# CreateIntelligens/index-tts-lora

Measured on AMD Instinct MI355X. Metric: audio-seconds/sec (RTF^-1) at batch 32, whole pipeline (GPT decode + latent pass + BigVGAN), higher is better.
Workload: dtype bf16; 1 GPU; BASELINE config 3: batch=32 utterances/GPU, top-k sampling (k=30,p=0.8), 140 acoustic tokens (5.97 s) each, shared 3.2 s prompt, text U{20..60} tokens, random-init weights at real shapes; gpt_dtype=bf16, vocoder_dtype=fp16, parallelism=dp1 (utterance sharding, no collectives), schedule=serial: one batch at a time on one stream

## Files before the change

index-tts-lora_amd/csrc/attention.hip:

```cpp
#include "common.h"
#include <type_traits>

namespace itts {

constexpr int HD = 64;

constexpr int AD_MAXCTX = 16384;
constexpr int AD_CH = 8;

__device__ __forceinline__ void softmax_merge(float& m, float& l, float m2, float l2, float& sa, float& sb) {
  float M = fmaxf(m, m2);
  sa = (m == -INFINITY) ? 0.f : __expf(m - M);
  sb = (m2 == -INFINITY) ? 0.f : __expf(m2 - M);
  l = l * sa + l2 * sb;
  m = M;
}

template <typename T, int NWV, bool IND, bool PAGED>
__global__ __launch_bounds__(NWV * 64) void attn_decode_kernel(const T* __restrict__ q, const T* __restrict__ kc,
                                                           const T* __restrict__ vc, T* __restrict__ out,
                                                           const int32_t* __restrict__ pad, const int32_t* __restrict__ pos,
                                                           int H, int smax, int out_mtp, const int32_t* __restrict__ kv_rows,
                                                           const int32_t* __restrict__ kv_step, int rows_total,
                                                           const int32_t* __restrict__ skip_rows,
                                                           const int32_t* __restrict__ kv_share,
                                                           const int32_t* __restrict__ kv_tab, int bs_log2) {
  typedef Elem<T> EL;
  typedef typename EL::frag frag;
  constexpr int E = EL::E;
  constexpr int LPR = HD / E;

  constexpr int RPW = 64 / LPR;
  constexpr int CH = AD_CH * 4 / NWV;
  __shared__ float w_m[NWV], w_l[NWV];
  __shared__ float w_o[NWV][HD];
  const int h = blockIdx.x, b = blockIdx.y;
  const int tid = threadIdx.x, lane = tid & 63, wave = tid >> 6;
  const int part = lane % LPR, rg = lane / LPR;
  const frag qv = ld16<frag>(q + ((int64_t)b * H + h) * HD + part * E);
  int tabv = 0, tab0v = 0;
  if constexpr (PAGED) {
    tabv = kv_tab[b * ITTS_KV_TAB + lane];
    tab0v = kv_tab[lane];
  }
  const int bsm = (1 << bs_log2) - 1;
  const int32_t* skip_ptr = skip_rows != nullptr ? skip_rows + b : pos;
  const int skip_raw = *skip_ptr;
  const int j0 = pad[b];
  const bool skipped = skip_rows != nullptr && skip_raw != 0;
  const int32_t* share_ptr = kv_share != nullptr ? kv_share : pos;
  const int share_raw = *share_ptr;
  const int share_w = (kv_share != nullptr && !IND) ? share_raw : 0;
  const int shC = share_w & 255;
  int pos0 = pos[0];
  asm volatile("" : "+s"(pos0));
  const int ctx = skipped ? j0 : pos0 + 1;
  const T* kb = kc + (PAGED ? 0 : ((int64_t)b * H + h) * smax * HD) + part * E;
  const T* vb = vc + (PAGED ? 0 : ((int64_t)b * H + h) * smax * HD) + part * E;
  const int64_t sh_off = ((int64_t)h * smax + (share_w >> 8)) * HD + part * E;
  const int32_t* tab = nullptr;
  if constexpr (IND) tab = kv_rows + ((int64_t)(kv_step[0] & 1) * rows_total + b) * smax;

  float qf[E];
  float m = -INFINITY, l = 0.f, o[E];
#pragma unroll
  for (int e = 0; e < E; ++e) o[e] = 0.f;

  const int wave_u = __builtin_amdgcn_readfirstlane(wave);
  auto key_pass = [&](const int base, auto first_tag) {
    constexpr bool FIRST = decltype(first_tag)::value;
    frag kf[CH], vf[CH];
    int prow[CH];
    if constexpr (IND) {
#pragma unroll
      for (int i = 0; i < CH; ++i) {
        int j = min(base + (i * NWV + wave) * RPW + rg, ctx - 1);
        prow[i] = tab[j];
      }
    }
#pragma unroll
    for (int i = 0; i < CH; ++i) {
      const int jf = min(base + (i * NWV + wave_u) * RPW, (ctx - 1) & ~(RPW - 1));
      int j = min(jf + rg, ctx - 1);
      int64_t ro = (int64_t)j * HD;
      if constexpr (IND) ro += (int64_t)(prow[i] - b) * H * smax * HD;
      if constexpr (PAGED) {
        const int blk = __builtin_amdgcn_readlane(tabv, (jf >> bs_log2) & (ITTS_KV_TAB - 1));
        ro = ((((int64_t)blk * H + h) << bs_log2) + (j & bsm)) * HD;
      }
      const T* kp = kb + ro;
      const T* vp = vb + ro;
      if constexpr (!IND) {
        const bool sh = (unsigned)(j - j0) < (unsigned)shC;
        int64_t so = sh_off + (int64_t)(j - j0) * HD;
        if constexpr (PAGED) {
          const int ps = (share_w >> 8) + (j - j0);
          const int blk0 = __shfl(tab0v, (ps >> bs_log2) & (ITTS_KV_TAB - 1), 64);
          so = ((((int64_t)blk0 * H + h) << bs_log2) + (ps & bsm)) * HD + part * E;
        }
        kp = sh ? kc + so : kp;
        vp = sh ? vc + so : vp;
      }
      kf[i] = ld16<frag>(kp);
      vf[i] = ld16<frag>(vp);
    }
    __builtin_amdgcn_sched_barrier(0);
    if constexpr (FIRST) {
#pragma unroll
      for (int e = 0; e < E; ++e) qf[e] = EL::to_f(qv[e]) * 0.125f;
      __builtin_amdgcn_sched_barrier(0);
    }
    float sc[CH];
    float cmax = -INFINITY;
#pragma unroll
    for (int i = 0; i < CH; ++i) {
      float d = 0.f;
#pragma unroll
      for (int e = 0; e < E; ++e) d = fmaf(qf[e], EL::to_f(kf[i][e]), d);
#pragma unroll
      for (int off = 1; off < LPR; off <<= 1) d += __shfl_xor(d, off, 64);
      int j = base + (i * NWV + wave) * RPW + rg;
      sc[i] = (j >= j0 && j < ctx) ? d : -INFINITY;
      cmax = fmaxf(cmax, sc[i]);
    }
    {
      const float M = fmaxf(m, cmax);
      const float Ms = (M == -INFINITY) ? 0.f : M;
      const float corr = (m == -INFINITY) ? 0.f : __expf(m - Ms);
      l *= corr;
#pragma unroll
      for (int e = 0; e < E; ++e) o[e] *= corr;
#pragma unroll
      for (int i = 0; i < CH; ++i) {
        float pv = __expf(sc[i] - Ms);
        l += pv;
#pragma unroll
        for (int e = 0; e < E; ++e) o[e] = fmaf(pv, EL::to_f(vf[i][e]), o[e]);
      }
      m = M;
    }
  };
  constexpr int PASS = 4 * RPW * AD_CH;
  if (j0 < ctx) {
    const int b0 = j0 & ~(RPW - 1);
    key_pass(b0, std::true_type{});
    for (int base = b0 + PASS; base < ctx; base += PASS) key_pass(base, std::false_type{});
  }
#pragma unroll
  for (int off = LPR; off < 64; off <<= 1) {
    float m2 = __shfl_xor(m, off, 64), l2 = __shfl_xor(l, off, 64);
    float sa, sb;
    softmax_merge(m, l, m2, l2, sa, sb);
#pragma unroll
    for (int e = 0; e < E; ++e) {
      float o2 = __shfl_xor(o[e], off, 64);
      o[e] = o[e] * sa + o2 * sb;
    }
  }
  if (rg == 0) {
#pragma unroll
    for (int e = 0; e < E; ++e) w_o[wave][part * E + e] = o[e];
    if (part == 0) {
      w_m[wave] = m;
      w_l[wave] = l;
    }
  }
  __syncthreads();
  if (tid < HD && !skipped) {
    float M = w_m[0];
#pragma unroll
    for (int w = 1; w < NWV; ++w) M = fmaxf(M, w_m[w]);
    float L = 0.f, acc = 0.f;
#pragma unroll
    for (int w = 0; w < NWV; ++w) {
      float sw = (w_m[w] == -INFINITY) ? 0.f : __expf(w_m[w] - M);
      L += w_l[w] * sw;
      acc += w_o[w][tid] * sw;
    }
    const int64_t o = out_mtp > 0 ? pa_off<T>(b, h * HD + tid, out_mtp) : ((int64_t)b * H + h) * HD + tid;
    out[o] = EL::from_f(L > 0.f ? acc / L : 0.f);
  }
}

template <typename T>
__global__ __launch_bounds__(256) void attn_prefill_kernel(const T* __restrict__ qkv, T* __restrict__ out,
                                                            T* __restrict__ kc, T* __restrict__ vc,
                                                            const int32_t* __restrict__ pad, int S, int H, int smax,
                                                            const int32_t* __restrict__ row_off,
                                                            const int32_t* __restrict__ cache_shift,
                                                            const T* __restrict__ pkc, const T* __restrict__ pvc,
                                                            const int32_t* __restrict__ pre_len,
                                                            const int32_t* __restrict__ pre_row,
                                                            const int32_t* __restrict__ pre_pos0, int pre_qkv,
                                                            T* wkc, T* wvc, const int32_t* __restrict__ w_row,
                                                            const int32_t* __restrict__ w_pos0,
                                                            const int32_t* __restrict__ kv_tab, int bs_log2) {
  typedef Elem<T> EL;
  typedef typename EL::frag frag;
  constexpr int E = EL::E, KS = EL::KS, NKS = HD / KS;
  constexpr int ES = (int)sizeof(T);
  constexpr int RS = HD * ES + 16;
  constexpr int CPR = HD / E;
  __shared__ __attribute__((aligned(16))) unsigned char Ks[64 * RS];
  __shared__ __attribute__((aligned(16))) unsigned char Vt[64 * RS];
  __shared__ __attribute__((aligned(16))) unsigned char Ps[4][16 * RS];
  const int q0 = blockIdx.x * 64, h = blockIdx.y, b = blockIdx.z;
  const int tid = threadIdx.x, lane = tid & 63, wave = tid >> 6;
  const int g = lane >> 4, c = lane & 15;
  const int D = H * HD;
  const int rbeg = row_off ? row_off[b] : b * S;
  if (row_off) S = row_off[b + 1] - rbeg;
  if (q0 >= S) return;
  const int cshift = (row_off && cache_shift) ? cache_shift[b] : 0;
  const int j0 = (pad && !row_off) ? pad[b] : 0;
  const T* base = qkv + (int64_t)rbeg * 3 * D;
  const int pl = pkc != nullptr ? pre_len[b] : 0;
  const int64_t pstr = pre_qkv ? (int64_t)3 * D : HD;
  const int64_t pbase = pkc == nullptr ? 0
                        : pre_qkv      ? (int64_t)pre_pos0[b] * 3 * D + h * HD
                                       : (((int64_t)pre_row[b] * H + h) * smax + pre_pos0[b]) * HD;
  const int p_row = (pkc != nullptr && !pre_qkv) ? pre_row[b] : 0, p_pos0 = (pkc != nullptr && !pre_qkv) ? pre_pos0[b] : 0;
  const int Stot = pl + S;
  if (wkc != nullptr) {
    const int wr = w_row[b], wp0 = w_pos0[b];
    for (int ch = tid; ch < 64 * CPR; ch += 256) {
      const int kk = ch / CPR, dc = ch - kk * CPR;
      const int q = q0 + kk;
      if (q < S) {
        const T* src = base + (int64_t)q * 3 * D + D + h * HD + dc * E;
        const int64_t o = kv_elem_off(kv_tab, bs_log2, wr, wp0 + q, H, h, smax) + dc * E;
        st16(wkc + o, ld16<frag>(src));
        st16(wvc + o, ld16<frag>(src + D));
      }
    }
  }

  frag qf[NKS];
  {
    const int row = q0 + wave * 16 + c;
#pragma unroll
    for (int ks = 0; ks < NKS; ++ks)
      qf[ks] = (row < S) ? ld16<frag>(base + (int64_t)row * 3 * D + h * HD + ks * KS + g * E) : zero_frag<frag>();
  }
  f32x4 O[4];
#pragma unroll
  for (int n = 0; n < 4; ++n) O[n] = f32x4{0.f, 0.f, 0.f, 0.f};
  float m[4], l[4];
#pragma unroll
  for (int j = 0; j < 4; ++j) { m[j] = -INFINITY; l[j] = 0.f; }

  const int jend = min(Stot, pl + q0 + 64);
  for (int jt = (j0 / 64) * 64; jt < jend; jt += 64) {
    __syncthreads();
    for (int ch = tid; ch < 64 * CPR; ch += 256) {
      const int kk = ch / CPR, dc = ch - kk * CPR;
      const int key = jt + kk;
      frag kv = zero_frag<frag>(), vv = zero_frag<frag>();
      if (key < pl) {
        const int64_t po = (kv_tab != nullptr && !pre_qkv) ? kv_elem_off(kv_tab, bs_log2, p_row, p_pos0 + key, H, h, smax) + dc * E
                                                           : pbase + (int64_t)key * pstr + dc * E;
        kv = ld16<frag>(pkc + po);
        vv = ld16<frag>(pvc + po);
      } else if (key < Stot) {
        const T* src = base + (int64_t)(key - pl) * 3 * D + D + h * HD + dc * E;
        kv = ld16<frag>(src);
        vv = ld16<frag>(src + D);
        if (kc != nullptr && jt == q0) {
          const int64_t o = kv_elem_off(kv_tab, bs_log2, b, key + cshift, H, h, smax) + dc * E;
          st16(kc + o, kv);
          st16(vc + o, vv);
        }
      }
      st16(Ks + kk * RS + dc * E * ES, kv);
#pragma unroll
      for (int e = 0; e < E; ++e) *reinterpret_cast<T*>(Vt + (dc * E + e) * RS + kk * ES) = vv[e];
    }
    __syncthreads();
    if (jt + 64 <= j0) continue;
    f32x4 sacc[4];
#pragma unroll
    for (int n = 0; n < 4; ++n) {
      sacc[n] = f32x4{0.f, 0.f, 0.f, 0.f};
#pragma unroll
      for (int ks = 0; ks < NKS; ++ks) {
        frag bf = ld16<frag>(Ks + (16 * n + c) * RS + (ks * KS + g * E) * ES);
        sacc[n] = EL::mma(qf[ks], bf, sacc[n]);
      }
    }
    float rmax[4];
#pragma unroll
    for (int j = 0; j < 4; ++j) {
      const int q = pl + q0 + wave * 16 + 4 * g + j;
      float mx = -INFINITY;
#pragma unroll
      for (int n = 0; n < 4; ++n) {
        const int key = jt + 16 * n + c;
        const bool vis = (key <= q) && (key >= j0) && (key < Stot);
        const float v = vis ? sacc[n][j] * 0.125f : -INFINITY;
        sacc[n][j] = v;
        mx = fmaxf(mx, v);
      }
#pragma unroll
      for (int o = 1; o < 16; o <<= 1) mx = fmaxf(mx, __shfl_xor(mx, o, 64));
      rmax[j] = mx;
    }
#pragma unroll
    for (int j = 0; j < 4; ++j) {
      const float mn = fmaxf(m[j], rmax[j]);
      const float corr = (m[j] == -INFINITY) ? 0.f : __expf(m[j] - mn);
      float rs = 0.f;
#pragma unroll
      for (int n = 0; n < 4; ++n) {
        const float pv = (sacc[n][j] == -INFINITY) ? 0.f : __expf(sacc[n][j] - mn);
        sacc[n][j] = pv;
        rs += pv;
      }
#pragma unroll
      for (int o = 1; o < 16; o <<= 1) rs += __shfl_xor(rs, o, 64);
      l[j] = l[j] * corr + rs;
      m[j] = mn;
#pragma unroll
      for (int n = 0; n < 4; ++n) O[n][j] *= corr;
    }
    unsigned char* ps = Ps[wave];
#pragma unroll
    for (int n = 0; n < 4; ++n)
#pragma unroll
      for (int j = 0; j < 4; ++j) *reinterpret_cast<T*>(ps + (4 * g + j) * RS + (16 * n + c) * ES) = EL::from_f(sacc[n][j]);
#pragma unroll
    for (int ks = 0; ks < NKS; ++ks) {
      frag af = ld16<frag>(ps + c * RS + (ks * KS + g * E) * ES);
#pragma unroll
      for (int n = 0; n < 4; ++n) {
        frag bf = ld16<frag>(Vt + (16 * n + c) * RS + (ks * KS + g * E) * ES);
        O[n] = EL::mma(af, bf, O[n]);
      }
    }
  }
#pragma unroll
  for (int j = 0; j < 4; ++j) {
    const int q = q0 + wave * 16 + 4 * g + j;
    if (q >= S) continue;
    const float inv = l[j] > 0.f ? 1.0f / l[j] : 0.f;
    T* orow = out + ((int64_t)rbeg + q) * D + h * HD;
#pragma unroll
    for (int n = 0; n < 4; ++n) orow[16 * n + c] = EL::from_f(O[n][j] * inv);
  }
}

}

using namespace itts;

#if ITTS_DIAG
namespace itts { int g_attn_waves = 4; }
#else
namespace itts { constexpr int g_attn_waves = 4; }
#endif

extern "C" int itts_attn_decode(const void* q, const void* kcache, const void* vcache, void* out, const int32_t* pad,
                                const int32_t* pos, int B, int H, int smax, int dtype, int out_packed, const int32_t* kv_rows,
                                const int32_t* kv_step, const int32_t* skip_rows, const int32_t* kv_share, const int32_t* kv_tab,
                                int kv_bs, void* stream) {
  const int out_mtp = out_packed ? (B + 15) / 16 : 0;
  ITTS_REQUIRE(q && kcache && vcache && out && pad && pos, "itts_attn_decode: null pointer");
  const bool paged = kv_tab != nullptr;
  ITTS_REQUIRE(B > 0 && H > 0 && (paged || (smax > 0 && smax <= AD_MAXCTX)), "itts_attn_decode: bad shape B=%d H=%d smax=%d (max %d)", B, H,
               smax, AD_MAXCTX);
  ITTS_REQUIRE(!paged || ((kv_bs == 16 || kv_bs == 32 || kv_bs == 64) && kv_rows == nullptr),
               "itts_attn_decode: a paged cache needs kv_bs in {16, 32, 64} and no beam row table");
  const int bs_log2 = kv_bs == 64 ? 6 : kv_bs == 32 ? 5 : 4;
  ITTS_REQUIRE((kv_rows == nullptr) == (kv_step == nullptr), "itts_attn_decode: pass both or neither of kv_rows / kv_step");
  hipStream_t s = (hipStream_t)stream;
  dim3 grid(H, B), block(g_attn_waves * 64);
  const bool ind = kv_rows != nullptr;
#define ITTS_AD(TT_, NW_, IND_, PG_)                                                                                        \
  hipLaunchKernelGGL((attn_decode_kernel<TT_, NW_, IND_, PG_>), grid, block, 0, s, (const TT_*)q, (const TT_*)kcache,      \
                     (const TT_*)vcache, (TT_*)out, pad, pos, H, smax, out_mtp, kv_rows, kv_step, B, skip_rows, kv_share, \
                     kv_tab, bs_log2)
#define ITTS_AD_T(TT_)                                                            \
  do {                                                                            \
    if (paged) { if (g_attn_waves == 8) ITTS_AD(TT_, 8, false, true); else ITTS_AD(TT_, 4, false, true); } \
    else if (g_attn_waves == 8) { if (ind) ITTS_AD(TT_, 8, true, false); else ITTS_AD(TT_, 8, false, false); } \
    else { if (ind) ITTS_AD(TT_, 4, true, false); else ITTS_AD(TT_, 4, false, false); }          \
  } while (0)
  switch (dtype) {
    case ITTS_F32:
      ITTS_AD_T(float);
      break;
    case ITTS_BF16:
      ITTS_AD_T(bf16_t);
      break;
    case ITTS_F16:
      ITTS_AD_T(f16_t);
      break;
    default:
      ITTS_REQUIRE(false, "itts_attn_decode: unknown dtype %d", dtype);
  }
#undef ITTS_AD_T
#undef ITTS_AD
  return check_launch("itts_attn_decode");
}

static int attn_prefill_impl(const void* qkv, void* out, void* kcache, void* vcache, const int32_t* pad, int B, int S, int H,
                             int smax, int dtype, const int32_t* row_off, const int32_t* cache_shift, void* stream,
                             const void* pkc = nullptr, const void* pvc = nullptr, const int32_t* pre_len = nullptr,
                             const int32_t* pre_row = nullptr, const int32_t* pre_pos0 = nullptr, int pre_qkv = 0,
                             void* wkc = nullptr, void* wvc = nullptr, const int32_t* w_row = nullptr,
                             const int32_t* w_pos0 = nullptr, const int32_t* kv_tab = nullptr, int kv_bs = 0) {
  ITTS_REQUIRE(qkv && out, "itts_attn_prefill: null pointer");
  ITTS_REQUIRE(kv_tab == nullptr || kv_bs == 16 || kv_bs == 32 || kv_bs == 64, "itts_attn_prefill: kv_bs must be 16, 32 or 64");
  const int bs_log2 = kv_bs == 64 ? 6 : kv_bs == 32 ? 5 : 4;
  if (kv_tab != nullptr && kcache != nullptr) smax = S > smax ? S : smax;
  ITTS_REQUIRE((kcache == nullptr) == (vcache == nullptr), "itts_attn_prefill: pass both caches or neither");
  ITTS_REQUIRE(B > 0 && S > 0 && H > 0 && (!kcache || S <= smax), "itts_attn_prefill: bad shape B=%d S=%d H=%d smax=%d", B, S, H, smax);
  ITTS_REQUIRE(B <= 65535 && H <= 65535, "itts_attn_prefill: grid too large");
  dim3 grid((S + 63) / 64, H, B), block(256);
  hipStream_t s = (hipStream_t)stream;
  switch (dtype) {
    case ITTS_F32:
      hipLaunchKernelGGL(attn_prefill_kernel<float>, grid, block, 0, s, (const float*)qkv, (float*)out, (float*)kcache, (float*)vcache, pad, S, H, smax, row_off, cache_shift,
                         (const float*)pkc, (const float*)pvc, pre_len, pre_row, pre_pos0, pre_qkv, (float*)wkc, (float*)wvc, w_row, w_pos0, kv_tab, bs_log2);
      break;
    case ITTS_BF16:
      hipLaunchKernelGGL(attn_prefill_kernel<bf16_t>, grid, block, 0, s, (const bf16_t*)qkv, (bf16_t*)out, (bf16_t*)kcache, (bf16_t*)vcache, pad, S, H, smax, row_off, cache_shift,
                         (const bf16_t*)pkc, (const bf16_t*)pvc, pre_len, pre_row, pre_pos0, pre_qkv, (bf16_t*)wkc, (bf16_t*)wvc, w_row, w_pos0, kv_tab, bs_log2);
      break;
    case ITTS_F16:
      hipLaunchKernelGGL(attn_prefill_kernel<f16_t>, grid, block, 0, s, (const f16_t*)qkv, (f16_t*)out, (f16_t*)kcache, (f16_t*)vcache, pad, S, H, smax, row_off, cache_shift,
                         (const f16_t*)pkc, (const f16_t*)pvc, pre_len, pre_row, pre_pos0, pre_qkv, (f16_t*)wkc, (f16_t*)wvc, w_row, w_pos0, kv_tab, bs_log2);
      break;
    default:
      ITTS_REQUIRE(false, "itts_attn_prefill: unknown dtype %d", dtype);
  }
  return check_launch("itts_attn_prefill");
}

extern "C" int itts_attn_prefill(const void* qkv, void* out, void* kcache, void* vcache, const int32_t* pad, int B, int S,
                                 int H, int smax, int dtype, void* stream) {
  return attn_prefill_impl(qkv, out, kcache, vcache, pad, B, S, H, smax, dtype, nullptr, nullptr, stream);
}

extern "C" int itts_attn_prefill_prefix(const void* qkv, void* out, const void* kcache, const void* vcache, const int32_t* row_off,
                                        const int32_t* pre_len, const int32_t* pre_row, const int32_t* pre_pos0, int B, int Smax,
                                        int H, int smax, int dtype, const int32_t* kv_tab, int kv_bs, void* stream) {
  ITTS_REQUIRE(row_off && kcache && vcache && pre_len && pre_row && pre_pos0, "itts_attn_prefill_prefix: null pointer");
  return attn_prefill_impl(qkv, out, nullptr, nullptr, nullptr, B, Smax, H, smax, dtype, row_off, nullptr, stream, kcache, vcache,
                           pre_len, pre_row, pre_pos0, 0, nullptr, nullptr, nullptr, nullptr, kv_tab, kv_bs);
}

extern "C" int itts_attn_prefill_shared(const void* qkv, void* out, void* kcache, void* vcache, const int32_t* row_off,
                                        const int32_t* pre_len, const int32_t* pre_row0, const int32_t* w_row,
                                        const int32_t* w_pos0, int E, int Smax, int H, int smax, int dtype, const int32_t* kv_tab,
                                        int kv_bs, void* stream) {
  ITTS_REQUIRE(qkv && row_off && pre_len && pre_row0 && (kcache == nullptr) == (vcache == nullptr) &&
                   (kcache == nullptr || (w_row && w_pos0)), "itts_attn_prefill_shared: null pointer");
  const int D = H * 64;
  const int es = dtype == ITTS_F32 ? 4 : 2;
  const char* q = (const char*)qkv;
  return attn_prefill_impl(qkv, out, nullptr, nullptr, nullptr, E, Smax, H, smax, dtype, row_off, nullptr, stream,
                           q + (int64_t)D * es, q + (int64_t)2 * D * es, pre_len, pre_len , pre_row0, 1, kcache, vcache,
                           w_row, w_pos0, kv_tab, kv_bs);
}

extern "C" int itts_attn_prefill_packed(const void* qkv, void* out, void* kcache, void* vcache, const int32_t* row_off,
                                        const int32_t* cache_shift, int B, int Smax, int H, int smax, int dtype,
                                        const int32_t* kv_tab, int kv_bs, void* stream) {
  ITTS_REQUIRE(row_off, "itts_attn_prefill_packed: row_off is null");
  return attn_prefill_impl(qkv, out, kcache, vcache, nullptr, B, Smax, H, smax, dtype, row_off, cache_shift, stream, nullptr, nullptr,
                           nullptr, nullptr, nullptr, 0, nullptr, nullptr, nullptr, nullptr, kv_tab, kv_bs);
}

namespace itts {
__global__ __launch_bounds__(256) void kv_share_rows_kernel(char* __restrict__ kc, char* __restrict__ vc, int64_t layer_bytes, int H, int C,
                                                            int p0, const int32_t* __restrict__ pad, int smax,
                                                            const int32_t* __restrict__ kv_tab, int bs_log2, int es, int total) {
  const int idx = (int)blockIdx.x * 256 + threadIdx.x;
  if (idx >= total) return;
  const int cpr = 64 * es / 16;
  const int seg = idx % cpr, kv = (idx / cpr) & 1, rest = idx / (2 * cpr);
  const int c = rest % C, h = rest / C;
  const int b = (int)blockIdx.y + 1;
  char* base = (kv ? vc : kc) + (int64_t)blockIdx.z * layer_bytes;
  const int64_t so = kv_elem_off(kv_tab, bs_log2, 0, p0 + c, H, h, smax) * es + seg * 16;
  const int64_t d_o = kv_elem_off(kv_tab, bs_log2, b, pad[b] + c, H, h, smax) * es + seg * 16;
  st16(base + d_o, ld16<B16>(base + so));
}
}

extern "C" int itts_kv_share_rows(void* kcache, void* vcache, int layers, int64_t layer_stride, int B, int H, int C, int p0,
                                  const int32_t* pad, int smax, const int32_t* kv_tab, int kv_bs, int dtype, void* stream) {
  ITTS_REQUIRE(kcache && vcache && pad && layers > 0 && B >= 1 && H > 0 && C > 0 && p0 >= 0, "itts_kv_share_rows: bad arguments");
  ITTS_REQUIRE(kv_tab != nullptr ? (kv_bs == 16 || kv_bs == 32 || kv_bs == 64) : smax >= p0 + C,
               "itts_kv_share_rows: paged cache: kv_bs must be 16, 32 or 64; contiguous cache: smax covers the block");
  ITTS_REQUIRE(layers <= 65535 && B <= 65536, "itts_kv_share_rows: too many layers / rows");
  if (B == 1) return ITTS_OK;
  const int es = dtype == ITTS_F32 ? 4 : 2;
  const int total = H * C * 2 * (64 * es / 16);
  hipLaunchKernelGGL(itts::kv_share_rows_kernel, dim3((total + 255) / 256, B - 1, layers), dim3(256), 0, (hipStream_t)stream, (char*)kcache,
                     (char*)vcache, layer_stride * es, H, C, p0, pad, smax, kv_tab, kv_bs == 64 ? 6 : kv_bs == 32 ? 5 : 4, es, total);
  return itts::check_launch("itts_kv_share_rows");
}
```

index-tts-lora_amd/csrc/gemm_skinny.hip:

```cpp
#include "common.h"
#include "ln_math.h"
#include <type_traits>

#ifndef ITTS_FOLD_ORDER
#define ITTS_FOLD_ORDER 0
#endif
#ifndef ITTS_NT_WEIGHTS
#define ITTS_NT_WEIGHTS 0
#endif

namespace itts {

template <typename F>
__device__ __forceinline__ F ldw(const void* p) {
  if constexpr (ITTS_NT_WEIGHTS) return ld16_nt<F>(p);
  else return ld16<F>(p);
}

struct SkinnyParams {
  int M, N, K;
  const void* wp;
  const float* bias;
  const void* x;
  int epi;
// ... 291 lines not shown
        f32x4 gv = {gelu_new(v[0]), gelu_new(v[1]), gelu_new(v[2]), gelu_new(v[3])};
        store4<T>((T*)p.y + (p.y_pa ? pa_off<T>(p.y_row0 + row, col0, p.y_mtp) : (int64_t)row * p.N + col0), gv, nval);
      } break;
      case ITTS_EPI_SILU_STORE: {
        f32x4 sv;
#pragma unroll
        for (int e = 0; e < 4; ++e) sv[e] = v[e] / (1.f + __expf(-v[e]));
        store4<T>((T*)p.y + (p.y_pa ? pa_off<T>(p.y_row0 + row, col0, p.y_mtp) : (int64_t)row * p.N + col0), sv, nval);
      } break;
      case ITTS_EPI_RELU_AFFINE_STORE:
      case ITTS_EPI_RELU_AFFINE_TANH_STORE: {
        const f32x4 sc = load4f(p.post_scale + col0, nval), sh = load4f(p.post_shift + col0, nval);
        f32x4 rv;
#pragma unroll
        for (int e = 0; e < 4; ++e) {
          rv[e] = fmaf(fmaxf(v[e], 0.f), sc[e], sh[e]);
          if (p.epi == ITTS_EPI_RELU_AFFINE_TANH_STORE) rv[e] = tanhf(rv[e]);
        }
        store4<T>((T*)p.y + (p.y_pa ? pa_off<T>(p.y_row0 + row, col0, p.y_mtp) : (int64_t)row * p.N + col0), rv, nval);
      } break;
      case ITTS_EPI_RESID_F32: {
        if constexpr (!FOLD) {
          const f32x4 nv = p2 + v;
          store4<float>(p.yf + (int64_t)row * p.N + col0, nv, nval);
          if (p.y != nullptr)
            store4<T>((T*)p.y + (p.y_pa ? pa_off<T>(p.y_row0 + row, col0, p.y_mtp) : (int64_t)row * p.N + col0), nv, nval);
        }
      } break;
      case ITTS_EPI_STORE_F32:
        store4<float>(p.yf + (int64_t)row * p.N + col0, v, nval);
        break;
      case ITTS_EPI_SLAB_F32:
        store4<float>(p.yf + ((int64_t)ks * p.slab_rows + row) * p.N + col0, v, nval);
        break;
      case ITTS_EPI_QKV_CACHE: {
        const int D = p.N / 3;
        if (col0 < D) {
          store4<T>((T*)p.y + (int64_t)row * D + col0, v, nval);
        } else {
          int cc = col0 - D;
          T* cache = (T*)(cc < D ? p.kcache : p.vcache);
          if (cc >= D) cc -= D;
          const int hh = cc >> 6, dd = cc & 63;
          const int64_t at = p.kv_tab == nullptr
                                 ? (((int64_t)row * p.heads + hh) * p.smax + pos_pre) * 64
                                 : ((((int64_t)blk * p.heads + hh) << p.kv_bs_log2) + (pos_pre & ((1 << p.kv_bs_log2) - 1))) * 64;
          store4<T>(cache + at + dd, v, nval);
        }
      } break;
    }
  };
#pragma unroll
  for (int ui = 0; ui < UPRE; ++ui) {
    const int u = wave + ui * NW;
    if (u < NTB * MT) unit(u, bias_pre[ui], pre2[ui], blk_pre[ui]);
  }
  for (int u = wave + UPRE * NW; u < NTB * MT; u += NW) {
    f32x4 bs = {0.f, 0.f, 0.f, 0.f}, p2 = bs;
    const int t = u / MT, mt = u - t * MT;
    const int col0 = (nt0 + t) * 16 + g * 4, row = (mt0 + mt) * 16 + r;
    if (col0 < p.N) {
      if (p.bias != nullptr && ks == 0) bs = load4f(p.bias + col0, p.N - col0);
      if constexpr (FOLD) p2 = load4f(p.cvec + col0, p.N - col0);
      else if (p.epi == ITTS_EPI_RESID_F32 && row < p.M) p2 = load4f(p.yf + (int64_t)row * p.N + col0, p.N - col0);
    }
    int blk = 0;
    if (p.kv_tab != nullptr && row < p.M)
      blk = p.kv_tab[(p.row0 + row) * ITTS_KV_TAB + ((pos_pre >> p.kv_bs_log2) & (ITTS_KV_TAB - 1))];
    unit(u, bs, p2, blk);
  }
  if (p.bump != nullptr && tid == 0 && (blockIdx.x | blockIdx.y | blockIdx.z) == 0) p.bump[0] += 1;
  ITTS_STAMP(5);
#if ITTS_STAMPS
  if (p.stamps != nullptr && threadIdx.x == 0) {
    ITTS_STAMP_DRAIN();
    unsigned long long te_;
    asm volatile("s_memtime %0\n\ts_waitcnt lgkmcnt(0)" : "=s"(te_)::"memory");
    unsigned xcc_;
    asm volatile("s_getreg_b32 %0, hwreg(HW_REG_XCC_ID)" : "=s"(xcc_));
    unsigned long long* o_ = p.stamps + (((size_t)blockIdx.z * gridDim.y + blockIdx.y) * gridDim.x + blockIdx.x) * 16;
#pragma unroll
    for (int i = 0; i < 10; ++i) o_[i] = st_[i];
    o_[10] = te_;
    o_[11] = rt0_;
    o_[12] = __builtin_amdgcn_s_memrealtime();
    o_[13] = xcc_ & 0xF;
  }
#endif
}

struct SkinnyPlan {
  int NW, spw, ntb, gx, gy, gz, SPWc, MT;
  size_t lds;
};

#if ITTS_DIAG
int g_tune_ntb = 0, g_tune_nw = 0;
int g_skinny_exp = 0;
#endif

template <typename T>
static SkinnyPlan plan_skinny(int N, int K, int ksplit, int MTall, int rows_per_wg, bool wide, bool fold) {
  constexpr int KS = Elem<T>::KS;
  SkinnyPlan q;
  int MT = MTall;
  if (rows_per_wg > 0 && rows_per_wg / 16 < MTall) MT = rows_per_wg / 16;
  const int gz = (MTall + MT - 1) / MT;
  const int KT = K / KS;
  const int SB = (KT + ksplit - 1) / ksplit;
  int NW = SB > 8 ? 8 : SB;
  if (wide && MT == 1 && SB > 80) NW = 16;
  if (NW < 1) NW = 1;
#if ITTS_DIAG
  if (g_tune_nw > 0) NW = g_tune_nw > 8 ? 8 : g_tune_nw;
#endif
  const int spw = (SB + NW - 1) / NW;
  const int NT = (N + 15) / 16;
  int ntb = (NT * ksplit * gz + 255) / 256;
#if ITTS_DIAG
  if (g_tune_ntb > 0) ntb = g_tune_ntb;
#endif
  const int SPWc = spw <= 5 ? 5 : 10;
  const int ntb_max = (fold && MT <= 2 && SPWc == 5) ? 4 : 3;
  if (ntb > ntb_max) ntb = ntb_max;
  if (SPWc == 10 && ntb > 2) ntb = 2;
  if (MT > 2 && SPWc == 10) ntb = 1;
  if (NW == 16) ntb = 1;
  if (fold && MT > 2 && ntb > 2) ntb = 2;
  q.NW = NW;
  q.spw = spw;
  q.ntb = ntb;
  q.SPWc = SPWc;
  q.MT = MT;
  q.gx = (NT + ntb - 1) / ntb;
  q.gy = ksplit;
  q.gz = gz;
  q.lds = (size_t)NW * ntb * MT * 256 * 4 + (fold ? (size_t)NW * MT * 32 * 4 : 0);
  if (q.lds < 1024) q.lds = 1024;
  return q;
}

template <typename T, int MT, bool FOLD>
static void launch_skinny_mt(const SkinnyParams& p, const SkinnyPlan& q, hipStream_t s) {
  dim3 grid(q.gx, q.gy, q.gz), block(q.NW * 64);
#define ITTS_SK(SPW_, NTB_, MAXW_) hipLaunchKernelGGL((gemm_skinny_kernel<T, MT, SPW_, NTB_, FOLD, MAXW_>), grid, block, q.lds, s, p)
  if constexpr (MT == 1 && !FOLD) {
    if (q.NW == 16) {
      ITTS_SK(10, 1, 16);
      return;
    }
  }
  if (q.SPWc == 5) {
    if (q.ntb == 1) ITTS_SK(5, 1, 8);
    else if (q.ntb == 2) ITTS_SK(5, 2, 8);
    else if (q.ntb == 3) {
      if constexpr (FOLD && MT > 2) ITTS_SK(5, 2, 8);
      else ITTS_SK(5, 3, 8);
    } else {
      if constexpr (FOLD && MT <= 2) ITTS_SK(5, 4, 8);
      else ITTS_SK(5, 1, 8);
    }
  } else {
    if (q.ntb == 1) ITTS_SK(10, 1, 8);
    else {
      if constexpr (MT <= 2) ITTS_SK(10, 2, 8);
      else ITTS_SK(10, 1, 8);
    }
  }
#undef ITTS_SK
}

template <typename T>
static int launch_skinny(const SkinnyParams& p, int rows_per_wg, bool wide, hipStream_t s) {
  const bool fold = p.cvec != nullptr;
  const int MTall = p.M <= 16 ? 1 : p.M <= 32 ? 2 : p.M <= 64 ? 4 : p.M <= 96 ? 6 : (p.M + 15) / 16;
  const SkinnyPlan q = plan_skinny<T>(p.N, p.K, p.ksplit, MTall, rows_per_wg, wide && !fold, fold);
  if constexpr (sizeof(T) == 4) {
    if (fold) {
      set_error("itts_gemm_skinny: the LayerNorm-folded form is built for bf16 / f16");
      return ITTS_ERR_INVALID;
    }
    launch_skinny_mt<T, 1, false>(p, q, s);
  } else {
#define ITTS_MT(MT_)                                          \
  do {                                                        \
    if (fold) launch_skinny_mt<T, MT_, true>(p, q, s);        \
    else launch_skinny_mt<T, MT_, false>(p, q, s);            \
  } while (0)
    if (q.MT == 1) ITTS_MT(1);
    else if (q.MT == 2) ITTS_MT(2);
    else if (q.MT == 4) ITTS_MT(4);
    else ITTS_MT(6);
#undef ITTS_MT
  }
  return check_launch("itts_gemm_skinny");
}

}

using namespace itts;

extern "C" int itts_gemm_skinny(const itts_skinny_args* a, void* stream) {
  ITTS_REQUIRE(a && a->wp && a->x, "itts_gemm_skinny: null args");
  const int ks = a->dtype == ITTS_F32 ? 16 : 32;
  const size_t esz = a->dtype == ITTS_F32 ? 4 : 2;
  ITTS_REQUIRE(a->M >= 0 && a->N > 0 && a->K > 0 && a->K % ks == 0, "itts_gemm_skinny: bad shape M=%d N=%d K=%d (K %% %d != 0)",
               a->M, a->N, a->K, ks);
  const int ksplit = a->ksplit > 0 ? a->ksplit : 1;
  ITTS_REQUIRE(ksplit <= a->K / ks && ksplit <= 64, "itts_gemm_skinny: ksplit=%d too large", ksplit);
  ITTS_REQUIRE(ksplit == 1 || a->epi == ITTS_EPI_SLAB_F32, "itts_gemm_skinny: ksplit > 1 requires the slab epilogue");
  if (a->epi == ITTS_EPI_QKV_CACHE)
    ITTS_REQUIRE(a->y && a->kcache && a->vcache && a->pos && a->N % 3 == 0 && a->N / 3 == a->heads * 64 &&
                     (a->kv_tab != nullptr ? (a->kv_bs == 16 || a->kv_bs == 32 || a->kv_bs == 64) : a->smax > 0),
                 "itts_gemm_skinny: bad QKV epilogue arguments (paged cache: kv_bs must be 16, 32 or 64)");
  else if (a->epi == ITTS_EPI_RESID_F32 || a->epi == ITTS_EPI_STORE_F32 || a->epi == ITTS_EPI_SLAB_F32)
    ITTS_REQUIRE(a->yf, "itts_gemm_skinny: yf is null");
  else
    ITTS_REQUIRE((a->epi == ITTS_EPI_STORE || a->epi == ITTS_EPI_GELU_STORE || a->epi == ITTS_EPI_SILU_STORE ||
                  a->epi == ITTS_EPI_RELU_AFFINE_STORE || a->epi == ITTS_EPI_RELU_AFFINE_TANH_STORE) && a->y,
                 "itts_gemm_skinny: bad epilogue %d", a->epi);
  if (a->epi == ITTS_EPI_RELU_AFFINE_STORE || a->epi == ITTS_EPI_RELU_AFFINE_TANH_STORE)
    ITTS_REQUIRE(a->post_scale && a->post_shift, "itts_gemm_skinny: the ReLU + affine epilogues need post_scale and post_shift");
  if (a->epi == ITTS_EPI_RESID_F32)
    ITTS_REQUIRE(a->N % 4 == 0 && (int64_t)a->M * a->N < (1ll << 29), "itts_gemm_skinny: the residual epilogue needs N %% 4 == 0");
  if (a->ln_c != nullptr)
    ITTS_REQUIRE(ksplit == 1 && a->bias && a->N % 4 == 0 && a->epi != ITTS_EPI_RESID_F32 && a->epi != ITTS_EPI_SLAB_F32 &&
                     a->dtype != ITTS_F32,
                 "itts_gemm_skinny: the LayerNorm-folded form needs ksplit 1, bias (= d), N %% 4 == 0, a storing epilogue, bf16 / f16");
  ITTS_REQUIRE(a->rows_per_wg == 0 || a->rows_per_wg == 16 || a->rows_per_wg == 32, "itts_gemm_skinny: rows_per_wg must be 0, 16 or 32");
  if (a->y_packed)
    ITTS_REQUIRE((a->epi == ITTS_EPI_STORE || a->epi == ITTS_EPI_GELU_STORE || a->epi == ITTS_EPI_SILU_STORE ||
                  a->epi == ITTS_EPI_RELU_AFFINE_STORE || a->epi == ITTS_EPI_RELU_AFFINE_TANH_STORE ||
                  a->epi == ITTS_EPI_RESID_F32) && a->N % ks == 0 && a->y,
                 "itts_gemm_skinny: a packed y needs the STORE / GELU_STORE / SILU_STORE / RESID_F32 epilogue and N %% %d == 0", ks);
  const int y_mtp = a->y_mtp > 0 ? a->y_mtp : (a->M + 15) / 16;
  ITTS_REQUIRE(a->y_row0 >= 0 && a->y_row0 % 16 == 0 && (!a->y_packed || a->y_row0 + a->M <= y_mtp * 16) &&
                   (a->y_packed || (a->y_row0 == 0 && a->y_mtp == 0)),
               "itts_gemm_skinny: y_row0 / y_mtp place the rows of a PACKED y inside a taller operand (y_row0 %% 16 == 0)");
  ITTS_REQUIRE(a->x_mtp == 0 || (a->x_packed && a->x_mtp * 16 >= a->M), "itts_gemm_skinny: x_mtp is for a packed x of at least M rows");
  if (a->M == 0) return ITTS_OK;
  const int rows_per = (a->dtype == ITTS_F32) ? 16 : (a->rows_per_wg > 0 ? (a->M > 96 ? a->M : 96) : 96);
  ITTS_REQUIRE(a->M <= 96 || a->rows_per_wg == 0 || (a->M + 15) / 16 / (a->rows_per_wg / 16) < 65535, "itts_gemm_skinny: too many rows");
  hipStream_t s = (hipStream_t)stream;
  for (int r0 = 0; r0 < a->M; r0 += rows_per) {
    SkinnyParams p;
    p.M = a->M - r0 < rows_per ? a->M - r0 : rows_per;
    p.N = a->N;
    p.K = a->K;
    p.wp = a->wp;
    p.bias = a->bias;
    p.x = a->x_packed ? (const char*)a->x : (const char*)a->x + (size_t)r0 * a->K * esz;
    p.x_pa = a->x_packed ? 1 : 0;
    p.y_pa = a->y_packed ? 1 : 0;
    p.mtp = a->x_mtp > 0 ? a->x_mtp : (a->M + 15) / 16;
    p.row0 = r0;
    p.y_mtp = y_mtp;
    p.post_scale = a->post_scale;
    p.post_shift = a->post_shift;
    p.y_row0 = r0 + a->y_row0;
    p.epi = a->epi;
    const size_t ycols = a->epi == ITTS_EPI_QKV_CACHE ? (size_t)a->N / 3 : (size_t)a->N;
    p.y = a->y ? (a->y_packed ? (char*)a->y : (char*)a->y + (size_t)r0 * ycols * esz) : nullptr;
    p.yf = a->yf ? a->yf + (size_t)r0 * a->N : nullptr;
    const size_t crow = (size_t)a->heads * a->smax * 64 * esz;
    const bool paged = a->kv_tab != nullptr;
    p.kcache = a->kcache ? (char*)a->kcache + (paged ? 0 : (size_t)r0 * crow) : nullptr;
    p.vcache = a->vcache ? (char*)a->vcache + (paged ? 0 : (size_t)r0 * crow) : nullptr;
    p.kv_tab = a->kv_tab;
    p.kv_bs_log2 = a->kv_bs == 64 ? 6 : a->kv_bs == 32 ? 5 : 4;
    p.pos = a->pos;
    p.heads = a->heads;
    p.smax = a->smax;
    p.ksplit = ksplit;
    p.slab_rows = a->M;
    p.cvec = a->ln_c;
    p.ln_eps = a->ln_eps > 0.f ? a->ln_eps : 1e-5f;
    p.bump = r0 == 0 ? a->bump : nullptr;
#if ITTS_STAMPS
    p.stamps = g_stamp_buf;
#endif
#if ITTS_DIAG
    p.exp = g_skinny_exp;
#endif
    int rc;
    if (a->dtype == ITTS_F32) rc = launch_skinny<float>(p, a->rows_per_wg, a->wide_wg != 0, s);
    else if (a->dtype == ITTS_BF16) rc = launch_skinny<bf16_t>(p, a->rows_per_wg, a->wide_wg != 0, s);
    else if (a->dtype == ITTS_F16) rc = launch_skinny<f16_t>(p, a->rows_per_wg, a->wide_wg != 0, s);
    else ITTS_REQUIRE(false, "itts_gemm_skinny: unknown dtype %d", a->dtype);
    if (rc != ITTS_OK) return rc;
  }
  return ITTS_OK;
}

extern "C" int itts_skinny_plan(int dtype, int M, int N, int K, int ksplit, int rows_per_wg, int wide_wg, int fold, int* out8) {
  ITTS_REQUIRE(out8 && N > 0 && K > 0 && ksplit > 0 && M > 0, "itts_skinny_plan: bad arguments");
  const int MT = dtype == ITTS_F32 ? 1 : M <= 16 ? 1 : M <= 32 ? 2 : M <= 64 ? 4 : (M <= 96 || rows_per_wg == 0) ? 6 : (M + 15) / 16;
  const SkinnyPlan q = dtype == ITTS_F32 ? plan_skinny<float>(N, K, ksplit, 1, 0, false, false)
                                         : plan_skinny<bf16_t>(N, K, ksplit, MT, rows_per_wg, wide_wg != 0 && !fold, fold != 0);
  out8[0] = q.gx; out8[1] = q.gy; out8[2] = q.NW; out8[3] = q.ntb; out8[4] = q.spw; out8[5] = (int)q.lds; out8[6] = q.gz; out8[7] = q.MT;
  return ITTS_OK;
}

#if ITTS_DIAG
namespace itts { extern int g_conv_cfg; extern int g_attn_waves; extern int g_conv_exp; }

extern "C" int itts_debug_set(int key, int value) {
  if (key == 1) itts::g_tune_ntb = value;
  else if (key == 2) itts::g_tune_nw = value;
  else if (key == 3) itts::g_conv_cfg = value;
  else if (key == 4) itts::g_attn_waves = (value == 8) ? 8 : 4;
  else if (key == 5) itts::g_conv_exp = value;
  else if (key == 6) itts::g_skinny_exp = value;
  else return ITTS_ERR_INVALID;
  return ITTS_OK;
}

extern "C" int itts_debug_stamps(void* buf) {
#if ITTS_STAMPS
  itts::g_stamp_buf = (unsigned long long*)buf;
  return ITTS_OK;
#else
  (void)buf;
  return ITTS_ERR_INVALID;
#endif
}

namespace itts { extern unsigned long long* g_stamp_buf_conv; }
extern "C" int itts_debug_stamps_conv(void* buf) {
#if ITTS_STAMPS
  itts::g_stamp_buf_conv = (unsigned long long*)buf;
  return ITTS_OK;
#else
  (void)buf;
  return ITTS_ERR_INVALID;
#endif
}

extern "C" int itts_debug_stamps_sample(void* buf) {
#if ITTS_STAMPS
  itts::g_stamp_buf_sample = (unsigned long long*)buf;
  return ITTS_OK;
#else
  (void)buf;
  return ITTS_ERR_INVALID;
#endif
}
#endif
```

Measured before the change: 1171 audio-seconds/sec.

## Size first attention decode pass to context length and split K/V load phases

For non-indexed 16-bit decode attention, the kernel now picks a first-pass chunk count (1/4, 1/2, 3/4 or full CH) from the actual context length. Short contexts therefore issue fewer K/V loads and less masked compute. K loads are now all issued before V loads, and the paged shared-prefix block lookups are hoisted ahead of the load loop. __syncthreads is replaced by an explicit lgkmcnt wait plus s_barrier. Diagnostic timestamp plumbing is added behind ITTS_DIAG/ITTS_STAMPS. The switch adds code size and possible register-pressure differences between template instantiations.

```diff
diff --git a/index-tts-lora_amd/csrc/attention.hip b/index-tts-lora_amd/csrc/attention.hip
--- a/index-tts-lora_amd/csrc/attention.hip
+++ b/index-tts-lora_amd/csrc/attention.hip
@@ -15,6 +15,32 @@
   l = l * sa + l2 * sb;
   m = M;
 }
+
+#if ITTS_DIAG
+#define ITTS_AD_DIAG_PARAMS , unsigned long long* __restrict__ stamps, int full_pass
+#define ITTS_AD_DIAG_ARGS , itts::g_stamp_buf_attn, itts::g_attn_full_pass
+unsigned long long* g_stamp_buf_attn = nullptr;
+int g_attn_full_pass = 0;
+#else
+#define ITTS_AD_DIAG_PARAMS
+#define ITTS_AD_DIAG_ARGS
+#endif
+#if ITTS_STAMPS
+#define AD_STAMP(i) ITTS_STAMP_IF(stamps != nullptr, i)
+#define AD_STAMP_LANDED(i, cnt)                                              \
+  do {                                                                       \
+    __builtin_amdgcn_sched_barrier(0);                                       \
+    if (stamps != nullptr && threadIdx.x == 0) {                             \
+      unsigned long long t_;                                                 \
+      asm volatile("s_waitcnt vmcnt(%1)\n\ts_memtime %0\n\ts_waitcnt lgkmcnt(0)" : "=s"(t_) : "n"(cnt) : "memory"); \
+      st_[i] = t_;                                                           \
+    }                                                                        \
+    __builtin_amdgcn_sched_barrier(0);                                       \
+  } while (0)
+#else
+#define AD_STAMP(i) do { } while (0)
+#define AD_STAMP_LANDED(i, cnt) do { } while (0)
+#endif
 
 template <typename T, int NWV, bool IND, bool PAGED>
 __global__ __launch_bounds__(NWV * 64) void attn_decode_kernel(const T* __restrict__ q, const T* __restrict__ kc,
@@ -24,7 +50,7 @@
                                                            const int32_t* __restrict__ kv_step, int rows_total,
                                                            const int32_t* __restrict__ skip_rows,
                                                            const int32_t* __restrict__ kv_share,
-                                                           const int32_t* __restrict__ kv_tab, int bs_log2) {
+                                                           const int32_t* __restrict__ kv_tab, int bs_log2 ITTS_AD_DIAG_PARAMS) {
   typedef Elem<T> EL;
   typedef typename EL::frag frag;
   constexpr int E = EL::E;
@@ -32,11 +58,18 @@
 
   constexpr int RPW = 64 / LPR;
   constexpr int CH = AD_CH * 4 / NWV;
+  constexpr bool SIZED = !IND && sizeof(T) == 2 && CH % 4 == 0;
   __shared__ float w_m[NWV], w_l[NWV];
   __shared__ float w_o[NWV][HD];
   const int h = blockIdx.x, b = blockIdx.y;
   const int tid = threadIdx.x, lane = tid & 63, wave = tid >> 6;
   const int part = lane % LPR, rg = lane / LPR;
+#if ITTS_STAMPS
+  __shared__ unsigned long long st_[16];
+  if (stamps != nullptr && tid < 16) st_[tid] = 0;
+  if (stamps != nullptr && tid == 0) st_[14] = __builtin_amdgcn_s_memrealtime();
+#endif
+  AD_STAMP(0);
   const frag qv = ld16<frag>(q + ((int64_t)b * H + h) * HD + part * E);
   int tabv = 0, tab0v = 0;
   if constexpr (PAGED) {
@@ -55,31 +88,44 @@
   int pos0 = pos[0];
   asm volatile("" : "+s"(pos0));
   const int ctx = skipped ? j0 : pos0 + 1;
-  const T* kb = kc + (PAGED ? 0 : ((int64_t)b * H + h) * smax * HD) + part * E;
-  const T* vb = vc + (PAGED ? 0 : ((int64_t)b * H + h) * smax * HD) + part * E;
+  const int64_t kboff = (PAGED ? 0 : ((int64_t)b * H + h) * smax * HD) + part * E;
   const int64_t sh_off = ((int64_t)h * smax + (share_w >> 8)) * HD + part * E;
   const int32_t* tab = nullptr;
   if constexpr (IND) tab = kv_rows + ((int64_t)(kv_step[0] & 1) * rows_total + b) * smax;
 
+  AD_STAMP(1);
+
   float qf[E];
   float m = -INFINITY, l = 0.f, o[E];
 #pragma unroll
   for (int e = 0; e < E; ++e) o[e] = 0.f;
 
   const int wave_u = __builtin_amdgcn_readfirstlane(wave);
-  auto key_pass = [&](const int base, auto first_tag) {
+  auto key_pass = [&](const int base, auto nch_tag, auto first_tag) {
+    constexpr int NCH = decltype(nch_tag)::value;
     constexpr bool FIRST = decltype(first_tag)::value;
-    frag kf[CH], vf[CH];
-    int prow[CH];
+    frag kf[NCH], vf[NCH];
+    int prow[NCH];
+    int64_t eo[NCH];
     if constexpr (IND) {
 #pragma unroll
-      for (int i = 0; i < CH; ++i) {
+      for (int i = 0; i < NCH; ++i) {
         int j = min(base + (i * NWV + wave) * RPW + rg, ctx - 1);
         prow[i] = tab[j];
       }
     }
-#pragma unroll
-    for (int i = 0; i < CH; ++i) {
+    int blk0[NCH];
+    if constexpr (PAGED && !IND) {
+#pragma unroll
+      for (int i = 0; i < NCH; ++i) {
+        const int jf = min(base + (i * NWV + wave_u) * RPW, (ctx - 1) & ~(RPW - 1));
+        const int ps = (share_w >> 8) + (min(jf + rg, ctx - 1) - j0);
+        blk0[i] = __shfl(tab0v, (ps >> bs_log2) & (ITTS_KV_TAB - 1), 64);
+      }
+      __builtin_amdgcn_sched_barrier(0);
+    }
+#pragma unroll
+    for (int i = 0; i < NCH; ++i) {
       const int jf = min(base + (i * NWV + wave_u) * RPW, (ctx - 1) & ~(RPW - 1));
       int j = min(jf + rg, ctx - 1);
       int64_t ro = (int64_t)j * HD;
@@ -88,32 +134,35 @@
         const int blk = __builtin_amdgcn_readlane(tabv, (jf >> bs_log2) & (ITTS_KV_TAB - 1));
         ro = ((((int64_t)blk * H + h) << bs_log2) + (j & bsm)) * HD;
       }
-      const T* kp = kb + ro;
-      const T* vp = vb + ro;
+      eo[i] = kboff + ro;
       if constexpr (!IND) {
         const bool sh = (unsigned)(j - j0) < (unsigned)shC;
         int64_t so = sh_off + (int64_t)(j - j0) * HD;
         if constexpr (PAGED) {
           const int ps = (share_w >> 8) + (j - j0);
-          const int blk0 = __shfl(tab0v, (ps >> bs_log2) & (ITTS_KV_TAB - 1), 64);
-          so = ((((int64_t)blk0 * H + h) << bs_log2) + (ps & bsm)) * HD + part * E;
+          so = ((((int64_t)blk0[i] * H + h) << bs_log2) + (ps & bsm)) * HD + part * E;
         }
-        kp = sh ? kc + so : kp;
-        vp = sh ? vc + so : vp;
-      }
-      kf[i] = ld16<frag>(kp);
-      vf[i] = ld16<frag>(vp);
-    }
+        asm("" : "+v"(so));
+        eo[i] = sh ? so : eo[i];
+      }
+      kf[i] = ld16<frag>(kc + eo[i]);
+    }
+    __builtin_amdgcn_sched_barrier(0);
+#pragma unroll
+    for (int i = 0; i < NCH; ++i) vf[i] = ld16<frag>(vc + eo[i]);
     __builtin_amdgcn_sched_barrier(0);
     if constexpr (FIRST) {
 #pragma unroll
       for (int e = 0; e < E; ++e) qf[e] = EL::to_f(qv[e]) * 0.125f;
       __builtin_amdgcn_sched_barrier(0);
-    }
-    float sc[CH];
+      AD_STAMP(2);
+      AD_STAMP_LANDED(3, 2 * NCH - 1);
+      AD_STAMP_LANDED(4, NCH);
+    }
+    float sc[NCH];
     float cmax = -INFINITY;
 #pragma unroll
-    for (int i = 0; i < CH; ++i) {
+    for (int i = 0; i < NCH; ++i) {
       float d = 0.f;
 #pragma unroll
       for (int e = 0; e < E; ++e) d = fmaf(qf[e], EL::to_f(kf[i][e]), d);
@@ -123,6 +172,7 @@
       sc[i] = (j >= j0 && j < ctx) ? d : -INFINITY;
       cmax = fmaxf(cmax, sc[i]);
     }
+    if constexpr (FIRST) AD_STAMP_LANDED(5, 0);
     {
       const float M = fmaxf(m, cmax);
       const float Ms = (M == -INFINITY) ? 0.f : M;
@@ -131,7 +181,7 @@
 #pragma unroll
       for (int e = 0; e < E; ++e) o[e] *= corr;
 #pragma unroll
-      for (int i = 0; i < CH; ++i) {
+      for (int i = 0; i < NCH; ++i) {
         float pv = __expf(sc[i] - Ms);
         l += pv;
 #pragma unroll
@@ -141,10 +191,29 @@
     }
   };
   constexpr int PASS = 4 * RPW * AD_CH;
+  typedef std::integral_constant<int, CH> full_t;
   if (j0 < ctx) {
     const int b0 = j0 & ~(RPW - 1);
-    key_pass(b0, std::true_type{});
-    for (int base = b0 + PASS; base < ctx; base += PASS) key_pass(base, std::false_type{});
+    int arm = SIZED ? __builtin_amdgcn_readfirstlane(min((ctx - b0 - 1) / (PASS / 4), 3)) : 3;
+#if ITTS_DIAG
+    if (full_pass) arm = 3;
+#endif
+    if constexpr (SIZED) {
+      switch (arm) {
+        case 0: key_pass(b0, std::integral_constant<int, CH / 4>{}, std::true_type{}); break;
+        case 1: key_pass(b0, std::integral_constant<int, CH / 2>{}, std::true_type{}); break;
+        case 2: key_pass(b0, std::integral_constant<int, 3 * CH / 4>{}, std::true_type{}); break;
+        default:
+          key_pass(b0, full_t{}, std::true_type{});
+          for (int base = b0 + PASS; base < ctx; base += PASS) key_pass(base, full_t{}, std::false_type{});
+      }
+    } else {
+      key_pass(b0, full_t{}, std::true_type{});
+      for (int base = b0 + PASS; base < ctx; base += PASS) key_pass(base, full_t{}, std::false_type{});
+    }
+#if ITTS_STAMPS
+    if (stamps != nullptr && tid == 0) st_[13] = (unsigned long long)((arm + 1) * CH / 4);
+#endif
   }
 #pragma unroll
   for (int off = LPR; off < 64; off <<= 1) {
@@ -165,7 +234,9 @@
       w_l[wave] = l;
     }
   }
-  __syncthreads();
+  asm volatile("s_waitcnt lgkmcnt(0)" ::: "memory");
+  __builtin_amdgcn_s_barrier();
+  asm volatile("" ::: "memory");
   if (tid < HD && !skipped) {
     float M = w_m[0];
 #pragma unroll
@@ -178,8 +249,17 @@
       acc += w_o[w][tid] * sw;
     }
     const int64_t o = out_mtp > 0 ? pa_off<T>(b, h * HD + tid, out_mtp) : ((int64_t)b * H + h) * HD + tid;
+    AD_STAMP(6);
     out[o] = EL::from_f(L > 0.f ? acc / L : 0.f);
   }
+  AD_STAMP(7);
+#if ITTS_STAMPS
+  if (stamps != nullptr && tid == 0) {
+    st_[12] = (unsigned long long)(j0 < ctx ? ctx - (j0 & ~(RPW - 1)) : 0);
+    st_[15] = __builtin_amdgcn_s_memrealtime();
+  }
+  if (stamps != nullptr && tid < 16) stamps[((size_t)blockIdx.y * gridDim.x + blockIdx.x) * 16 + tid] = st_[tid];
+#endif
 }
 
 template <typename T>
@@ -377,7 +457,7 @@
 #define ITTS_AD(TT_, NW_, IND_, PG_)                                                                                        \
   hipLaunchKernelGGL((attn_decode_kernel<TT_, NW_, IND_, PG_>), grid, block, 0, s, (const TT_*)q, (const TT_*)kcache,      \
                      (const TT_*)vcache, (TT_*)out, pad, pos, H, smax, out_mtp, kv_rows, kv_step, B, skip_rows, kv_share, \
-                     kv_tab, bs_log2)
+                     kv_tab, bs_log2 ITTS_AD_DIAG_ARGS)
 #define ITTS_AD_T(TT_)                                                            \
   do {                                                                            \
     if (paged) { if (g_attn_waves == 8) ITTS_AD(TT_, 8, false, true); else ITTS_AD(TT_, 4, false, true); } \
diff --git a/index-tts-lora_amd/csrc/gemm_skinny.hip b/index-tts-lora_amd/csrc/gemm_skinny.hip
--- a/index-tts-lora_amd/csrc/gemm_skinny.hip
+++ b/index-tts-lora_amd/csrc/gemm_skinny.hip
@@ -617,7 +617,8 @@
 }
 
 #if ITTS_DIAG
-namespace itts { extern int g_conv_cfg; extern int g_attn_waves; extern int g_conv_exp; }
+namespace itts { extern int g_conv_cfg; extern int g_attn_waves; extern int g_conv_exp; extern int g_attn_full_pass;
+                 extern unsigned long long* g_stamp_buf_attn; int g_stamp_target = 0; }
 
 extern "C" int itts_debug_set(int key, int value) {
   if (key == 1) itts::g_tune_ntb = value;
@@ -626,13 +627,16 @@
   else if (key == 4) itts::g_attn_waves = (value == 8) ? 8 : 4;
   else if (key == 5) itts::g_conv_exp = value;
   else if (key == 6) itts::g_skinny_exp = value;
+  else if (key == 7) itts::g_attn_full_pass = value != 0;
+  else if (key == 8) itts::g_stamp_target = value == 1;
   else return ITTS_ERR_INVALID;
   return ITTS_OK;
 }
 
 extern "C" int itts_debug_stamps(void* buf) {
 #if ITTS_STAMPS
-  itts::g_stamp_buf = (unsigned long long*)buf;
+  if (itts::g_stamp_target == 1) itts::g_stamp_buf_attn = (unsigned long long*)buf;
+  else itts::g_stamp_buf = (unsigned long long*)buf;
   return ITTS_OK;
 #else
   (void)buf;
```

Measured after the change: 1186 audio-seconds/sec (median of 6 runs). 1.3% higher.
